# revdotcom/reverb

Hardware: NVIDIA H100
Metric: rtfx_attention_rescoring_30s_chunks (higher is better)
Workload: dtype bf16

## Files before the change

### include/rvb_b200.h

```cpp
#ifndef RVB_B200_H_
#define RVB_B200_H_

#if defined(__GNUC__)
#define RVB_API __attribute__((visibility("default")))
#else
#define RVB_API
#endif

#ifdef __cplusplus
extern "C" {
#endif

typedef struct rvb_model rvb_model;

typedef struct rvb_model_config {
  int input_dim;
  int d_model;
  int heads;
  int ffn_dim;
  int num_blocks;
  int cnn_kernel;
  int causal;
  int cnn_layer_norm;
  int num_langs;
// ... 87 lines not shown
RVB_API int rvb_decoder_step_topk(rvb_model* m, const float* d_enc_out, const int* h_enc_lens, int B, int Tp, int N,
                                  const int* h_hyps, int L, const float* h_cat_embs, int n_cat, int k, float* h_topk_val,
                                  int* h_topk_idx, void* stream);

RVB_API int rvb_decoder_cache_begin(rvb_model* m, const float* d_enc_out, const int* h_enc_lens, int B, int Tp, int N,
                                    int max_steps, const float* h_cat_embs, int n_cat, void* stream);
RVB_API int rvb_decoder_cache_step(rvb_model* m, const int* h_tokens, const int* h_parents, int k, float* h_topk_val,
                                   int* h_topk_idx, void* stream);
RVB_API int rvb_decoder_cache_end(rvb_model* m);

RVB_API int rvb_decoder_step_logp(rvb_model* m, const float* d_enc_out, const int* h_enc_lens, int B, int Tp, int N,
                                  const int* h_hyps, int L, const float* h_cat_embs, int n_cat, float* h_logp,
                                  void* stream);

RVB_API int rvb_ctc_force_align(const float* d_logp, int V, const int* h_enc_lens, int B, int Tp, const int* h_labels,
                                const int* h_label_lens, int max_U, int blank_id, int* h_frames, int* h_first,
                                int* h_last, int* h_peak, float* h_peak_logp, float* h_score, double* h_loglik,
                                void* stream);

typedef struct rvb_aligner rvb_aligner;
RVB_API long long rvb_aligner_workspace_bytes(int U, int total_frames, int want_loglik);
RVB_API rvb_aligner* rvb_aligner_begin(rvb_model* m, const int* h_labels, int U, int total_frames, int V, int blank_id,
                                       int want_loglik, long long budget_bytes, void* stream);
RVB_API int rvb_aligner_push(rvb_aligner* a, const float* d_logp, int n_rows, void* stream);
RVB_API int rvb_aligner_finish(rvb_aligner* a, int* h_frames, int* h_first, int* h_last, int* h_peak, float* h_peak_logp,
                               float* h_score, double* h_loglik, void* stream);
RVB_API void rvb_aligner_abort(rvb_aligner* a);

RVB_API int rvb_gemm_bf16(const void* d_A, const void* d_W, const float* d_bias, int M, int N, int K, int act, int out_mode,
                  float alpha, void* d_out, int ldo, void* stream);
RVB_API int rvb_gemm_bf16_rows(const void* d_A, const void* d_W, const float* d_bias, int M, int N, int K, int act,
                               int out_mode, float alpha, void* d_out, int ldo, const int* d_row_lens, int rows_per_batch,
                               void* stream);
RVB_API int rvb_gemm_bf16x3(const void* d_A, const void* d_W, const float* d_bias, int M, int N, int K, int act, int out_mode,
                            float alpha, void* d_out, int ldo, void* stream);
RVB_API int rvb_gemm_grouped(const void* d_A, const void* d_W, const float* d_bias, int M, int N, int K, int out_mode,
                             void* d_out, int ldo, const int* d_grp, int rows_per_batch, int group_n, int x3,
                             void* stream);
RVB_API int rvb_f32_to_bf16_pair(const float* d_x, void* d_out, long long rows, int width, void* stream);
RVB_API long long rvb_gemm_logsoftmax_gather_ws_bytes(int M, int N);
RVB_API int rvb_gemm_logsoftmax_gather(const void* d_A, const void* d_W, const float* d_bias, int M, int N, int K,
                                       const int* d_gather, void* d_ws, float* d_out, void* stream);
RVB_API int rvb_layernorm(const float* d_x, const float* d_gamma, const float* d_beta, float eps, int M, int d,
                  void* d_out_bf16, float* d_out_f32, void* stream);
RVB_API int rvb_attention(const void* d_q, const void* d_k, const void* d_v, const void* d_p, const float* d_bias_u,
                  const float* d_bias_v, void* d_out, int ldq, int ldk, int ldv, int ldp, int ldo, int Bq, int Tq, int Tk,
                  int H, int dk, int q_per_kv, const int* d_k_lens, const int* d_q_lens, int causal, float scale,
                  void* stream);
RVB_API int rvb_attention_tc(const void* d_q, const void* d_k, const void* d_v, void* d_out, int ldq, int ldk, int ldv,
                             int ldo, int groups, int Tq, int Tk, int H, int dk, const float* d_key_bias,
                             const int* d_k_lens, int causal, float scale, void* stream);
RVB_API int rvb_attention_tc_chunked(const void* d_q, const void* d_k, const void* d_v, void* d_out, int ldq, int ldk,
                                     int ldv, int ldo, int groups, int Tq, int Tk, int H, int dk, const float* d_key_bias,
                                     const int* d_k_lens, int chunk, int left_chunks, float scale, void* stream);
RVB_API int rvb_attention_tc_bits(const void* d_q, const void* d_k, const void* d_v, void* d_out, int ldq, int ldk,
                                  int ldv, int ldo, int groups, int Tq, int Tk, int H, int dk, const float* d_key_bias,
                                  const int* d_k_lens, int causal, const void* d_key_bits, int bits_ld, float scale,
                                  void* stream);
RVB_API int rvb_attention_tc_blocks_per_sm(int Tk, int causal, int chunk, int with_key_bits);
RVB_API int rvb_relpos_prep(const void* d_k, int ldk, const void* d_pos, int ldp, const float* d_bias_u,
                            const float* d_bias_v, void* d_kpp, float* d_cbias, int B, int T, int H, int dk,
                            void* stream);
RVB_API int rvb_f32_to_bf16(const float* d_x, void* d_out, long long n, void* stream);

typedef struct rvb_flac_info {
  int sample_rate;
// ... 30 lines not shown
```

### reverb_b200/_lib.py

```python
from __future__ import annotations

import ctypes as C
import os
from typing import Optional

_HERE = os.path.dirname(os.path.abspath(__file__))
LIB_PATH = os.environ.get("RVB_LIB_PATH") or os.path.join(_HERE, "librvb_b200.so")


class ModelConfig(C.Structure):
    _fields_ = [(n, C.c_int) for n in (
        "input_dim", "d_model", "heads", "ffn_dim", "num_blocks", "cnn_kernel", "causal",
        "cnn_layer_norm", "num_langs", "vocab", "dec_heads", "dec_ffn_dim", "dec_blocks", "r_dec_blocks",
        "sos_id", "eos_id", "precision")]


class SegConfig(C.Structure):
    _fields_ = [(n, C.c_int) for n in (
        "sample_rate", "sinc_filters", "sinc_kernel", "sinc_stride", "conv_channels", "conv_kernel", "lstm_hidden",
        "lstm_layers", "linear_dim", "linear_layers", "num_classes")]


class WavlmSegConfig(C.Structure):
    _fields_ = [(n, C.c_int) for n in (
# ... 40 lines not shown
    "rvb_encoder_forward": (_i, [_vp, _vp, _vp, _i, _i, _vp, _i, _vp, _vp, _vp]),
    "rvb_encoder_forward_chunked": (_i, [_vp, _vp, _vp, _i, _i, _vp, _i, _i, _i, _vp, _vp, _vp]),
    "rvb_encoder_forward_streaming": (_i, [_vp, _vp, _i, _i, _vp, _i, _i, _i, _vp, _vp, _vp]),
    "rvb_ctc_topk": (_i, [_vp, _vp, _i, _i, _i, _f, _i, _vp, _vp, _vp, _vp]),
    "rvb_logp_topk": (_i, [_vp, _i, _i, _i, _vp, _vp, _vp]),
    "rvb_ctc_greedy_search": (_i, [_vp, _i, _vp, _i, _i, _i, _vp, _vp, _vp]),
    "rvb_resample": (_i, [_vp, _i, _ll, _vp, _i, _i, _i, _vp, _ll, _vp]),
    "rvb_ctc_prefix_beam_search": (_i, [_vp, _vp, _i, _vp, _i, _i, _i, _i, _i, _vp, _vp, _vp, _vp, _vp, _vp]),
    "rvb_beam_search_rescoring": (_i, [_vp, _vp, _vp, _i, _vp, _vp, _i, _i, _i, _i, _vp, _i, _f, _i, _vp, _vp, _vp, _vp, _vp,
                                       _vp, _vp, _vp, _vp]),
    "rvb_search_submit": (_i, [_vp, _vp, _vp, _i, _vp, _vp, _i, _i, _i, _i, _vp]),
    "rvb_search_submit_biased": (_i, [_vp, _vp, _vp, _i, _vp, _vp, _i, _i, _i, _i, _vp, _vp]),
    "rvb_context_graph_create": (_vp, [_i, _vp, _vp, _vp, _vp, _vp, _vp, _vp, _i, _i]),
    "rvb_context_graph_destroy": (None, [_vp]),
    "rvb_ctc_prefix_beam_search_biased": (_i, [_vp, _vp, _i, _vp, _i, _i, _i, _i, _i, _vp, _vp, _vp, _vp, _vp, _vp,
                                               _vp]),
    "rvb_rescoring_submit": (_i, [_vp, _i, _vp, _i, _f, _i, _i, _vp, _vp, _vp, _vp, _vp, _vp]),
    "rvb_rescoring_collect": (_i, [_vp, _i, _vp, _vp, _vp]),
    "rvb_ticket_release": (_i, [_vp, _i]),
    "rvb_decoder_step_topk": (_i, [_vp, _vp, _vp, _i, _i, _i, _vp, _i, _vp, _i, _i, _vp, _vp, _vp]),
    "rvb_decoder_cache_begin": (_i, [_vp, _vp, _vp, _i, _i, _i, _i, _vp, _i, _vp]),
    "rvb_decoder_cache_step": (_i, [_vp, _vp, _vp, _i, _vp, _vp, _vp]),
    "rvb_decoder_cache_end": (_i, [_vp]),
    "rvb_decoder_step_logp": (_i, [_vp, _vp, _vp, _i, _i, _i, _vp, _i, _vp, _i, _vp, _vp]),
    "rvb_attention_rescoring": (_i, [_vp, _vp, _vp, _i, _i, _vp, _vp, _i, _i, _vp, _i, _f, _vp, _vp, _vp]),
    "rvb_ctc_force_align": (_i, [_vp, _i, _vp, _i, _i, _vp, _vp, _i, _i, _vp, _vp, _vp, _vp, _vp, _vp, _vp, _vp]),
    "rvb_aligner_workspace_bytes": (_ll, [_i, _i, _i]),
    "rvb_aligner_begin": (_vp, [_vp, _vp, _i, _i, _i, _i, _i, _ll, _vp]),
    "rvb_aligner_push": (_i, [_vp, _vp, _i, _vp]),
    "rvb_aligner_finish": (_i, [_vp, _vp, _vp, _vp, _vp, _vp, _vp, _vp, _vp]),
    "rvb_aligner_abort": (None, [_vp]),
    "rvb_gemm_bf16": (_i, [_vp, _vp, _vp, _i, _i, _i, _i, _i, _f, _vp, _i, _vp]),
    "rvb_gemm_bf16_rows": (_i, [_vp, _vp, _vp, _i, _i, _i, _i, _i, _f, _vp, _i, _vp, _i, _vp]),
    "rvb_gemm_bf16x3": (_i, [_vp, _vp, _vp, _i, _i, _i, _i, _i, _f, _vp, _i, _vp]),
    "rvb_gemm_grouped": (_i, [_vp, _vp, _vp, _i, _i, _i, _i, _vp, _i, _vp, _i, _i, _i, _vp]),
    "rvb_f32_to_bf16_pair": (_i, [_vp, _vp, _ll, _i, _vp]),
    "rvb_gemm_logsoftmax_gather_ws_bytes": (_ll, [_i, _i]),
    "rvb_gemm_logsoftmax_gather": (_i, [_vp, _vp, _vp, _i, _i, _i, _vp, _vp, _vp, _vp]),
    "rvb_layernorm": (_i, [_vp, _vp, _vp, _f, _i, _i, _vp, _vp, _vp]),
    "rvb_attention": (_i, [_vp, _vp, _vp, _vp, _vp, _vp, _vp, _i, _i, _i, _i, _i, _i, _i, _i, _i, _i, _i, _vp, _vp,
                           _i, _f, _vp]),
    "rvb_attention_tc_chunked": (_i, [_vp, _vp, _vp, _vp, _i, _i, _i, _i, _i, _i, _i, _i, _i, _vp, _vp, _i, _i, _f, _vp]),
    "rvb_attention_tc": (_i, [_vp, _vp, _vp, _vp, _i, _i, _i, _i, _i, _i, _i, _i, _i, _vp, _vp, _i, _f, _vp]),
    "rvb_attention_tc_bits": (_i, [_vp, _vp, _vp, _vp, _i, _i, _i, _i, _i, _i, _i, _i, _i, _vp, _vp, _i, _vp, _i, _f,
                                   _vp]),
    "rvb_attention_tc_blocks_per_sm": (_i, [_i, _i, _i, _i]),
    "rvb_relpos_prep": (_i, [_vp, _i, _vp, _i, _vp, _vp, _vp, _vp, _i, _i, _i, _i, _vp]),
    "rvb_f32_to_bf16": (_i, [_vp, _vp, _ll, _vp]),
    "rvb_flac_index_workspace_bytes": (_ll, [_ll]),
    "rvb_flac_index": (_i, [_vp, _ll, _ll, C.POINTER(FlacInfo), _vp, _ll, _vp, _vp, _vp]),
    "rvb_flac_decode_workspace_bytes": (_ll, [_i, _ll, C.POINTER(FlacInfo)]),
    "rvb_flac_decode": (_i, [_vp, _ll, C.POINTER(FlacInfo), _vp, _i, _ll, _vp, _ll, _vp, _vp, _vp, _vp, _vp]),
    "rvb_wav_decode": (_i, [_vp, _ll, C.POINTER(WavCodec), _ll, _vp, _vp, _vp, _vp]),
    "rvb_seg_create": (_vp, [C.POINTER(SegConfig)]),
    "rvb_seg_set_tensor": (_i, [_vp, C.c_char_p, _vp, _ll]),
    "rvb_seg_finalize": (_i, [_vp]),
    "rvb_seg_destroy": (None, [_vp]),
    "rvb_seg_num_frames": (_i, [_vp, _i]),
    "rvb_seg_forward": (_i, [_vp, _vp, _i, _i, _vp, _vp, _vp]),
    "rvb_wavlm_seg_create": (_vp, [C.POINTER(WavlmSegConfig)]),
    "rvb_wavlm_seg_set_tensor": (_i, [_vp, C.c_char_p, _vp, _ll]),
    "rvb_wavlm_seg_finalize": (_i, [_vp]),
    "rvb_wavlm_seg_destroy": (None, [_vp]),
    "rvb_wavlm_seg_num_frames": (_i, [_vp, _i]),
    "rvb_wavlm_seg_forward": (_i, [_vp, _vp, _i, _i, _vp, _vp, _vp, _vp]),
    "rvb_attention_tc_relbias": (_i, [_vp, _vp, _vp, _vp, _i, _i, _i, _i, _i, _i, _i, _vp, _vp, _f, _vp]),
# ... 41 lines not shown
```

### reverb_b200/csrc/engine.cu

```cuda
#include <math.h>
#include <stdarg.h>
#include <stdlib.h>
#include <string.h>

#include <algorithm>
#include <atomic>
#include <memory>
#include <string>
#include <vector>

#include "../../include/rvb_b200.h"
#include "host_mem.h"
#include "kernels.h"

namespace rvb {

static thread_local char g_err[1024] = "";
std::atomic<unsigned long long> g_launch_count{0};
void set_error(const char* fmt, ...) {
  va_list ap;
  va_start(ap, fmt);
  vsnprintf(g_err, sizeof(g_err), fmt, ap);
  va_end(ap);
}
// ... 1881 lines not shown
  g.W = reinterpret_cast<const rvb::bf16*>(d_W);
  g.M = M;
  g.N = N;
  g.K = K;
  g.bias = d_bias;
  g.act = act;
  g.out_mode = out_mode;
  g.alpha = alpha;
  g.out = d_out;
  g.ldo = ldo;
  return rvb::launch_gemm(g, (cudaStream_t)stream);
}

RVB_API int rvb_gemm_bf16_rows(const void* d_A, const void* d_W, const float* d_bias, int M, int N, int K, int act,
                               int out_mode, float alpha, void* d_out, int ldo, const int* d_row_lens, int rows_per_batch,
                               void* stream) {
  rvb::GemmArgs g;
  g.A = reinterpret_cast<const rvb::bf16*>(d_A);
  g.W = reinterpret_cast<const rvb::bf16*>(d_W);
  g.M = M;
  g.N = N;
  g.K = K;
  g.bias = d_bias;
  g.act = act;
  g.out_mode = out_mode;
  g.alpha = alpha;
  g.out = d_out;
  g.ldo = ldo;
  g.row_lens = d_row_lens;
  g.rows_per_batch = rows_per_batch;
  return rvb::launch_gemm(g, (cudaStream_t)stream);
}

RVB_API int rvb_gemm_bf16x3(const void* d_A, const void* d_W, const float* d_bias, int M, int N, int K, int act, int out_mode,
                            float alpha, void* d_out, int ldo, void* stream) {
  rvb::GemmArgs g;
  g.A = reinterpret_cast<const rvb::bf16*>(d_A);
  g.W = reinterpret_cast<const rvb::bf16*>(d_W);
  g.M = M;
  g.N = N;
  g.K = K;
  g.bias = d_bias;
  g.act = act;
  g.out_mode = out_mode;
  g.alpha = alpha;
  g.out = d_out;
  g.ldo = ldo;
  g.x3 = 1;
  if (out_mode == rvb::OUT_BF16) g.out_split = (act == rvb::ACT_GLU) ? N / 2 : N;
  return rvb::launch_gemm(g, (cudaStream_t)stream);
}

RVB_API int rvb_gemm_grouped(const void* d_A, const void* d_W, const float* d_bias, int M, int N, int K, int out_mode,
                             void* d_out, int ldo, const int* d_grp, int rows_per_batch, int group_n, int x3,
                             void* stream) {
  rvb::GemmArgs g;
  g.A = reinterpret_cast<const rvb::bf16*>(d_A);
  g.W = reinterpret_cast<const rvb::bf16*>(d_W);
  g.M = M;
  g.N = N;
  g.K = K;
  g.bias = d_bias;
  g.out_mode = out_mode;
  g.out = d_out;
  g.ldo = ldo;
  g.grp = d_grp;
// ... 138 lines not shown
```

### reverb_b200/csrc/gemm.cu

```cuda
#include <cuda.h>
#include <stdlib.h>
#include <string.h>

#include <algorithm>
#include <mutex>
#include <vector>

#include "kernels.h"

namespace rvb {

static int g_gemm_impl = -1;
void set_gemm_impl(int impl) { g_gemm_impl = impl; }
int get_gemm_impl() {
  if (g_gemm_impl < 0) {
    const char* e = getenv("RVB_GEMM");
    g_gemm_impl = (e && strcmp(e, "simt") == 0) ? 1 : (e && strcmp(e, "narrow") == 0) ? 2 : 0;
  }
  return g_gemm_impl;
}

struct GemmKParams {
  int M, N, K, num_k_blocks;
  int tiles_n, num_tiles;
// ... 232 lines not shown
  }
}

__device__ __forceinline__ long long output_row(const GemmKParams& p, const TileCoord& t, int r) {
  if (p.conv_mode) {
    int tp = t.row0 + r;
    if (tp >= p.conv_T2) return -1;
    return ((long long)t.b * p.conv_T2 + tp) * p.conv_orow_mul + t.f;
  }
  int m = t.row0 + r;
  if (m >= p.M) return -1;
  if (p.row_lens != nullptr) {
    int b = m / p.rows_per_batch;
    int pos = m - b * p.rows_per_batch;
    if (pos >= __ldg(p.row_lens + b)) return -1;
  }
  if (p.grp != nullptr && __ldg(p.grp + m / p.rows_per_batch) != t.g) return -1;
  return m;
}

template <int BN>
__device__ __forceinline__ void acc_ld32(const float* accs, int row, int c, uint32_t* r) {
  const float* rp = accs + row * BN;
#pragma unroll
  for (int k = 0; k < 8; ++k) {
    const float4 v = *reinterpret_cast<const float4*>(rp + ((((c >> 2) + k) ^ (row & 7)) << 2));
    r[4 * k + 0] = __float_as_uint(v.x);
    r[4 * k + 1] = __float_as_uint(v.y);
    r[4 * k + 2] = __float_as_uint(v.z);
    r[4 * k + 3] = __float_as_uint(v.w);
  }
}

template <int BN, int EPI, bool PAIR>
__device__ __forceinline__ void drain_tile(const GemmKParams& p, const TileCoord& t, int q, int lane, const float* accs,
                                           int c0, int c1, float* stage) {
  const int arow = q * 32 + lane;
  const long long orow = output_row(p, t, arow);
  const int n0_tile = t.n0;
  const int oshift = t.g * p.group_n;
  if (p.debug_skip_epi == 1) return;
  if constexpr (EPI == EPI_LSE) {
    const int g = (orow >= 0) ? __ldg(p.lse_gather + orow) : -1;
#pragma unroll 1
    for (int cs = c0; cs < c1; cs += 128) {
      float m = -INFINITY, ssum = 0.f;
#pragma unroll 1
      for (int c = cs; c < cs + 128 && c < c1; c += 32) {
        const int n0 = n0_tile + c;
        if (n0 >= p.N) break;
        uint32_t acc[32];
        acc_ld32<BN>(accs, arow, c, acc);
        float x[32];
        float cm = -INFINITY;
        if (n0 + 32 <= p.N && p.bias != nullptr && (reinterpret_cast<uintptr_t>(p.bias) & 15) == 0) {
          const float2 one2 = make_float2(1.f, 1.f);
          float mx[4] = {-INFINITY, -INFINITY, -INFINITY, -INFINITY};
#pragma unroll
          for (int j = 0; j < 8; ++j) {
            const float4 b4 = __ldg(reinterpret_cast<const float4*>(p.bias + n0) + j);
            const float2 lo = ffma2(make_float2(__uint_as_float(acc[4 * j]), __uint_as_float(acc[4 * j + 1])), one2,
                                    make_float2(b4.x, b4.y));
            const float2 hi = ffma2(make_float2(__uint_as_float(acc[4 * j + 2]), __uint_as_float(acc[4 * j + 3])), one2,
                                    make_float2(b4.z, b4.w));
            x[4 * j] = lo.x;
            x[4 * j + 1] = lo.y;
// ... 159 lines not shown
          float v[8];
          const float2 one2 = make_float2(1.f, 1.f);
#pragma unroll
          for (int h = 0; h < 2; ++h) {
            float4 b4 = make_float4(0.f, 0.f, 0.f, 0.f);
            if (p.bias != nullptr) b4 = __ldg(reinterpret_cast<const float4*>(p.bias + n0) + 2 * j + h);
            float2 lo = ffma2(make_float2(__uint_as_float(acc[8 * j + 4 * h + 0]), __uint_as_float(acc[8 * j + 4 * h + 1])),
                              one2, make_float2(b4.x, b4.y));
            float2 hi = ffma2(make_float2(__uint_as_float(acc[8 * j + 4 * h + 2]), __uint_as_float(acc[8 * j + 4 * h + 3])),
                              one2, make_float2(b4.z, b4.w));
            if (EPI == EPI_BF16_SILU) {
              if constexpr (PAIR) {
                lo = make_float2(lo.x / (1.f + expf(-lo.x)), lo.y / (1.f + expf(-lo.y)));
                hi = make_float2(hi.x / (1.f + expf(-hi.x)), hi.y / (1.f + expf(-hi.y)));
              } else {
                lo = gated2(lo, lo);
                hi = gated2(hi, hi);
              }
            }
            v[4 * h + 0] = lo.x;
            v[4 * h + 1] = lo.y;
            v[4 * h + 2] = hi.x;
            v[4 * h + 3] = hi.y;
          }
          if (EPI == EPI_BF16_RELU) {
#pragma unroll
            for (int e = 0; e < 8; ++e) v[e] = fmaxf(v[e], 0.f);
          }
          if (EPI == EPI_BF16_GELU) {
#pragma unroll
            for (int e = 0; e < 8; ++e) v[e] = gelu_erf(v[e]);
          }
          if constexpr (EPI == EPI_BF16_RELPOS) {
            if (kcols) {
              const uint4 pv = *reinterpret_cast<const uint4*>(p.rp_pos + (long long)rp_t * p.rp_ldp + rp_hc + 8 * j);
              const float4 u0 = __ldg(reinterpret_cast<const float4*>(p.rp_u + rp_hc + 8 * j));
              const float4 u1 = __ldg(reinterpret_cast<const float4*>(p.rp_u + rp_hc + 8 * j) + 1);
              const float uu[8] = {u0.x, u0.y, u0.z, u0.w, u1.x, u1.y, u1.z, u1.w};
              const float4 v0 = __ldg(reinterpret_cast<const float4*>(p.rp_v + rp_hc + 8 * j));
              const float4 v1 = __ldg(reinterpret_cast<const float4*>(p.rp_v + rp_hc + 8 * j) + 1);
              const float2 p0 = unpack_bf16x2(pv.x), p1 = unpack_bf16x2(pv.y), p2 = unpack_bf16x2(pv.z), p3 = unpack_bf16x2(pv.w);
              const float pp[8] = {p0.x, p0.y, p1.x, p1.y, p2.x, p2.y, p3.x, p3.y};
              float kq[8];
#pragma unroll
              for (int e = 0; e < 8; ++e) {
                kq[e] = __bfloat162float(__float2bfloat16(v[e]));
                v[e] = kq[e] + pp[e];
              }
              rp_part[j] = uu[0] * kq[0] + uu[1] * kq[1] + uu[2] * kq[2] + uu[3] * kq[3] + uu[4] * kq[4] + uu[5] * kq[5] +
                           uu[6] * kq[6] + uu[7] * kq[7] + v0.x * pp[0] + v0.y * pp[1] + v0.z * pp[2] + v0.w * pp[3] +
                           v1.x * pp[4] + v1.y * pp[5] + v1.z * pp[6] + v1.w * pp[7];
            }
          }
          if (PAIR && part == 1) {
#pragma unroll
            for (int e = 0; e < 8; ++e) v[e] -= __bfloat162float(__float2bfloat16(v[e]));
          }
          if (p.debug_skip_epi == 3 && v[0] != 123.456f) continue;
          *reinterpret_cast<uint4*>(stage_u + lane * 32 + ((j ^ (lane & 7)) << 2)) =
              make_uint4(pack_bf16x2(v[0], v[1]), pack_bf16x2(v[2], v[3]), pack_bf16x2(v[4], v[5]),
                         pack_bf16x2(v[6], v[7]));
        }
        if (p.debug_skip_epi == 3) continue;
        __syncwarp();
#pragma unroll
        for (int it = 0; it < 8; ++it) {
          const int row = it * 4 + rsub;
          const uint4 u = *reinterpret_cast<const uint4*>(stage_u + row * 32 + ((slot ^ (row & 7)) << 2));
          if (ro[it] >= 0 && p.debug_skip_epi != 2)
            *reinterpret_cast<uint4*>(out + ro[it] + c + (PAIR ? part * p.out_split : 0)) = u;
        }
        __syncwarp();
        }
        if constexpr (EPI == EPI_BF16_RELPOS) {
          if (kcols && orow >= 0) {
            const int hh = rp_hc >> 6;
            p.rp_cb[((orow / p.rp_T) * p.rp_H + hh) * (long long)p.rp_T + rp_t] =
                ((rp_part[0] + rp_part[4]) + (rp_part[2] + rp_part[6])) + ((rp_part[1] + rp_part[5]) + (rp_part[3] + rp_part[7]));
          }
        }
      } else {
        for (int cc = c; cc < c + 64 && cc < c1; cc += 32) {
          if (n0_tile + cc >= p.N) break;
          uint32_t acc[32];
          acc_ld32<BN>(accs, arow, cc, acc);
// ... 208 lines not shown
        if (prev >= 0 && lane == 0) mbar_arrive(&empty[prev]);
        prev = (int)stage;
        if (++stage == STAGES) {
          stage = 0;
          phase ^= 1;
        }
      }
      mbar_arrive(&turn[wg ^ 1]);
      wgmma_wait<0>();
      wgmma_fence_regs<BN>(acc);
      if (prev >= 0 && lane == 0) mbar_arrive(&empty[prev]);
      if (i > 0) mbar_wait(&accfree[wg], hand_parity);
#pragma unroll
      for (int h = 0; h < 2; ++h) {
        const int r0 = h * 64 + wl * 16 + (lane >> 2);
#pragma unroll
        for (int j = 0; j < BN / 8; ++j) {
          const int c = 8 * j + 2 * (lane & 3);
#pragma unroll
          for (int e = 0; e < 2; ++e) {
            const int r = r0 + 8 * e;
            *reinterpret_cast<float2*>(accs + r * BN + ((((c >> 2)) ^ (r & 7)) << 2) + (c & 3)) =
                make_float2(acc[h * (BN / 2) + 4 * j + 2 * e], acc[h * (BN / 2) + 4 * j + 2 * e + 1]);
          }
        }
      }
      asm volatile("bar.sync %0, 128;" ::"r"(1 + wg) : "memory");
      drain_tile<BN, EPI, PAIR>(p, t, wl, lane, accs, 0, BN, stage_w);
      mbar_arrive(&accfree[wg ^ 1]);
    }
  }
}

struct WideCfg {
  static constexpr int BM = 128;
  static constexpr int BN = 256;
  static constexpr int BK = 64;
  static constexpr int STAGES = 3;
  static constexpr uint32_t A_BYTES = BM * BK * 2;
  static constexpr uint32_t B_BYTES = BN * BK * 2;
  static constexpr uint32_t STAGE_BYTES = A_BYTES + B_BYTES;
  static constexpr uint32_t OUT_BYTES = BM * BN * 2;
  static constexpr uint32_t SMEM_BYTES = STAGES * STAGE_BYTES + OUT_BYTES + 256  + 1024 ;
};

template <int EPI>
__global__ void __launch_bounds__(kGemmThreads, 1)
gemm_wide_kernel(const __grid_constant__ CUtensorMap tmA, const __grid_constant__ CUtensorMap tmB, const GemmKParams p) {
  using Cfg = WideCfg;
  constexpr int STAGES = Cfg::STAGES;
  extern __shared__ uint8_t smem_raw[];
  uint8_t* smem = reinterpret_cast<uint8_t*>((reinterpret_cast<uintptr_t>(smem_raw) + 1023) & ~uintptr_t(1023));
  uint8_t* sA = smem;
  uint8_t* sB = smem + STAGES * Cfg::A_BYTES;
  uint8_t* sOut = smem + STAGES * Cfg::STAGE_BYTES;
  uint64_t* bars = reinterpret_cast<uint64_t*>(sOut + Cfg::OUT_BYTES);
  uint64_t* full = bars;
  uint64_t* empty = bars + STAGES;
  uint64_t* ofull = bars + 2 * STAGES;
  uint64_t* ofree = ofull + 1;

  const int warp = threadIdx.x >> 5;
  const int lane = threadIdx.x & 31;

  if (threadIdx.x == 0) {
    for (int i = 0; i < STAGES; ++i) {
      mbar_init(&full[i], 1);
      mbar_init(&empty[i], 8);
    }
    mbar_init(ofull, 256);
    mbar_init(ofree, 96);
    fence_barrier_init();
    tma_prefetch_desc(&tmA);
    tma_prefetch_desc(&tmB);
  }
  __syncthreads();
  const int nkb = p.num_k_blocks;

  if (warp < 4) {
    setmaxnreg_dec<kProducerRegs>();
    if (warp == 0) {
      if (lane == 0) {
        uint32_t stage = 0, phase = 0;
        for (int tile = blockIdx.x; tile < p.num_tiles; tile += gridDim.x) {
          const TileCoord t = decode_tile(p, tile, Cfg::BN);
          for (int kb = 0; kb < nkb; ++kb) {
            mbar_wait(&empty[stage], phase ^ 1);
            mbar_expect_tx(&full[stage], Cfg::STAGE_BYTES);
            if (p.conv_mode) {
              const int tap = kb / p.conv_cblocks;
              const int cb = kb - tap * p.conv_cblocks;
              const int kh = tap / 3, kw = tap - kh * 3;
              tma_load_4d(sA + stage * Cfg::A_BYTES, &tmA, &full[stage], cb * 64, 2 * t.f + kw, t.row0 + (kh >> 1),
                          t.b * 2 + (kh & 1));
            } else {
              tma_load_4d(sA + stage * Cfg::A_BYTES, &tmA, &full[stage], kb * 64, t.row0, 0, 0);
            }
            tma_load_2d(sB + stage * Cfg::B_BYTES, &tmB, &full[stage], kb * 64, t.n0);
            if (++stage == STAGES) {
              stage = 0;
              phase ^= 1;
            }
          }
        }
      }
    } else {
      const int cw = warp - 1;
      const bool store = p.debug_skip_epi == 0;
      bf16* out = reinterpret_cast<bf16*>(p.out);
      int i = 0;
      for (int tile = blockIdx.x; tile < p.num_tiles; tile += gridDim.x, ++i) {
        const TileCoord t = decode_tile(p, tile, Cfg::BN);
        mbar_wait(ofull, i & 1);
        if (store) {
#pragma unroll 4
          for (int r = cw; r < Cfg::BM; r += 3) {
            const long long orow = output_row(p, t, r);
            const uint4 u = *reinterpret_cast<const uint4*>(sOut + r * (Cfg::BN * 2) + ((lane ^ (r & 7)) << 4));
            if (orow >= 0) *reinterpret_cast<uint4*>(out + orow * p.ldo + t.n0 + lane * 8) = u;
          }
        }
        mbar_arrive(ofree);
      }
    }
  } else {
    setmaxnreg_inc<kConsumerRegs>();
    const int wg = (warp >> 2) - 1, wl = warp & 3;
    float acc[Cfg::BN / 2];
    uint32_t stage = 0, phase = 0;
    int i = 0;
    for (int tile = blockIdx.x; tile < p.num_tiles; tile += gridDim.x, ++i) {
      const TileCoord t = decode_tile(p, tile, Cfg::BN);
#pragma unroll
      for (int e = 0; e < Cfg::BN / 2; ++e) acc[e] = 0.f;
      int prev = -1;
      for (int kb = 0; kb < nkb; ++kb) {
        mbar_wait(&full[stage], phase);
        constexpr uint64_t kHalfA = (Cfg::A_BYTES / 2) >> 4;
        const uint64_t adesc = make_sw128_desc(smem_u32(sA + stage * Cfg::A_BYTES)) + wg * kHalfA;
        const uint64_t bdesc = make_sw128_desc(smem_u32(sB + stage * Cfg::B_BYTES));
        wgmma_fence_regs<Cfg::BN / 2>(acc);
        wgmma_fence();
#pragma unroll
        for (int k = 0; k < 4; ++k) wgmma_m64n256k16_ss(acc, adesc + 2 * k, bdesc + 2 * k, 1u);
        wgmma_commit();
        wgmma_wait<1>();
        wgmma_fence_regs<Cfg::BN / 2>(acc);
        if (prev >= 0 && lane == 0) mbar_arrive(&empty[prev]);
        prev = (int)stage;
        if (++stage == STAGES) {
          stage = 0;
          phase ^= 1;
        }
      }
      wgmma_wait<0>();
      wgmma_fence_regs<Cfg::BN / 2>(acc);
      if (lane == 0) mbar_arrive(&empty[prev]);
      if (i > 0) mbar_wait(ofree, (i - 1) & 1);
      if (p.debug_skip_epi != 1) {
        const int r0 = wg * 64 + wl * 16 + (lane >> 2);
        uint32_t* so = reinterpret_cast<uint32_t*>(sOut) + r0 * (Cfg::BN / 2) + (lane & 3);
        const float2 one2 = make_float2(1.f, 1.f);
#pragma unroll
        for (int j = 0; j < Cfg::BN / 8; ++j) {
          float2 b = make_float2(0.f, 0.f);
          if (p.bias != nullptr) b = __ldg(reinterpret_cast<const float2*>(p.bias + t.n0 + 8 * j + 2 * (lane & 3)));
#pragma unroll
          for (int e = 0; e < 2; ++e) {
            float2 v = ffma2(make_float2(acc[4 * j + 2 * e], acc[4 * j + 2 * e + 1]), one2, b);
            if (EPI == EPI_BF16_SILU) v = gated2(v, v);
            if (EPI == EPI_BF16_RELU) v = make_float2(fmaxf(v.x, 0.f), fmaxf(v.y, 0.f));
            so[8 * e * (Cfg::BN / 2) + ((j ^ (lane >> 2)) << 2)] = pack_bf16x2(v.x, v.y);
          }
        }
      }
      mbar_arrive(ofull);
    }
  }
}

__device__ __forceinline__ float load_a_elem(const GemmKParams& p, const TileCoord& t, int r, int k) {
  if (k >= p.K) return 0.0f;
  if (p.conv_mode) {
    int tp = t.row0 + r;
    if (tp >= p.conv_T2) return 0.0f;
    int tap = k / p.conv_C;
    int c = k - tap * p.conv_C;
    int kh = tap / 3, kw = tap - kh * 3;
    long long idx = (((long long)(t.b * 2 + (kh & 1)) * p.conv_T1h + (tp + (kh >> 1))) * p.conv_F1 + (2 * t.f + kw)) *
                        p.conv_C + c;
    return __bfloat162float(p.A[idx]);
  }
  int m = t.row0 + r;
  if (m >= p.M) return 0.0f;
  return __bfloat162float(p.A[(long long)m * p.lda + k]);
}

__global__ void __launch_bounds__(256) gemm_simt_kernel(const GemmKParams p) {
  __shared__ float sA[128][17];
  __shared__ float sW[32][17];
  __shared__ float sG[32][17];
  const bool glu = (p.act == ACT_GLU);
  for (int tile = blockIdx.x; tile < p.num_tiles; tile += gridDim.x) {
    TileCoord t = decode_tile(p, tile, 32);
    const int tx = threadIdx.x & 7, ty = threadIdx.x >> 3;
// ... 115 lines not shown
    cudaEvent_t e;
    RVB_CHECK_CUDA(cudaEventCreate(&e));
    pool.push_back(e);
  }
  *out = pool[g_prof_pool_used[dev]++];
  return 0;
}

void gemm_profile_begin() {
  std::lock_guard<std::mutex> lock(g_prof_mutex);
  g_prof.clear();
  for (int d = 0; d < kProfMaxDev; ++d) g_prof_pool_used[d] = 0;
  g_prof_on = true;
}
int gemm_profile_end(double* total_ms, double* total_flops, long long* launches) {
  g_prof_on = false;
  double ms = 0.0, fl = 0.0;
  for (auto& r : g_prof) {
    float t = 0.f;
    RVB_CHECK_CUDA(cudaEventSynchronize(r.b));
    RVB_CHECK_CUDA(cudaEventElapsedTime(&t, r.a, r.b));
    ms += t;
    fl += r.flops;
  }
  if (total_ms) *total_ms = ms;
  if (total_flops) *total_flops = fl;
  if (launches) *launches = (long long)g_prof.size();
  g_prof.clear();
  return 0;
}

template <int BN>
static int launch_wg(const GemmArgs& a, GemmKParams& p, cudaStream_t stream) {
  constexpr uint32_t SMEM_BYTES = BN == 256 ? WideCfg::SMEM_BYTES : GemmCfg<BN>::SMEM_BYTES;
  CUtensorMap tmA, tmB;
  const int kmul = a.x3 ? 2 : 1;
  const long long lda = a.lda ? a.lda : (long long)a.K * kmul, ldw = a.ldw ? a.ldw : (long long)a.K * kmul;
  if (a.conv_mode) {
    const cuuint64_t Cp = (cuuint64_t)a.conv_C * (a.x3 ? 2 : 1);
    cuuint64_t dims[4] = {Cp, (cuuint64_t)a.conv_F1, (cuuint64_t)a.conv_T1h, (cuuint64_t)(2 * a.conv_B)};
    cuuint64_t str[3] = {Cp * 2, (cuuint64_t)a.conv_F1 * Cp * 2, (cuuint64_t)a.conv_T1h * a.conv_F1 * Cp * 2};
    cuuint32_t box[4] = {64, 1, 128, 1};
    if (make_tmap(&tmA, a.A, 4, dims, str, box)) return -1;
  } else {
    cuuint64_t dims[4] = {(cuuint64_t)a.K * (a.x3 ? 2 : 1), (cuuint64_t)a.M, 1, 1};
    cuuint64_t str[3] = {(cuuint64_t)lda * 2, (cuuint64_t)lda * 2 * a.M, (cuuint64_t)lda * 2 * a.M};
    cuuint32_t box[4] = {64, 128, 1, 1};
    if (make_tmap(&tmA, a.A, 4, dims, str, box)) return -1;
  }
  {
    cuuint64_t dims[2] = {(cuuint64_t)a.K * (a.x3 ? 2 : 1), (cuuint64_t)a.N};
    cuuint64_t str[1] = {(cuuint64_t)ldw * 2};
    cuuint32_t box[2] = {64, (cuuint32_t)BN};
    if (make_tmap(&tmB, a.W, 2, dims, str, box)) return -1;
  }
  void (*kern)(const CUtensorMap, const CUtensorMap, const GemmKParams) = nullptr;
  if constexpr (BN == 256) {
    switch (select_epi(a.act, a.out_mode)) {
      case EPI_BF16: kern = gemm_wide_kernel<EPI_BF16>; break;
      case EPI_BF16_RELU: kern = gemm_wide_kernel<EPI_BF16_RELU>; break;
      default: kern = gemm_wide_kernel<EPI_BF16_SILU>; break;
    }
  } else {
    const bool pair = a.out_split > 0;
    switch (a.rp_pos ? (int)EPI_BF16_RELPOS : select_epi(a.act, a.out_mode)) {
      case EPI_BF16: kern = pair ? gemm_wg_kernel<BN, EPI_BF16, true> : gemm_wg_kernel<BN, EPI_BF16, false>; break;
      case EPI_BF16_RELU: kern = pair ? gemm_wg_kernel<BN, EPI_BF16_RELU, true> : gemm_wg_kernel<BN, EPI_BF16_RELU, false>; break;
      case EPI_BF16_SILU: kern = pair ? gemm_wg_kernel<BN, EPI_BF16_SILU, true> : gemm_wg_kernel<BN, EPI_BF16_SILU, false>; break;
      case EPI_F32: kern = gemm_wg_kernel<BN, EPI_F32, false>; break;
      case EPI_RESID: kern = gemm_wg_kernel<BN, EPI_RESID, false>; break;
      case EPI_GLU: kern = pair ? gemm_wg_kernel<BN, EPI_GLU, true> : gemm_wg_kernel<BN, EPI_GLU, false>; break;
      case EPI_LSE: kern = gemm_wg_kernel<BN, EPI_LSE, false>; break;
      case EPI_BF16_RELPOS: kern = gemm_wg_kernel<BN, EPI_BF16_RELPOS, false>; break;
      case EPI_BF16_GELU: kern = gemm_wg_kernel<BN, EPI_BF16_GELU, false>; break;
      default: kern = gemm_wg_kernel<BN, EPI_GENERIC, false>; break;
    }
  }
  RVB_CHECK_CUDA(cudaFuncSetAttribute(kern, cudaFuncAttributeMaxDynamicSharedMemorySize, (int)SMEM_BYTES));
  p.tiles_n = a.grp ? p.grp_slots * (p.group_n / BN) : (a.N + BN - 1) / BN;
  int tiles_m = a.conv_mode ? a.conv_B * a.conv_F2 * p.conv_tt : (a.M + 127) / 128;
  p.num_tiles = tiles_m * p.tiles_n;
  int grid = p.num_tiles < g_num_sms ? p.num_tiles : g_num_sms;
  GemmProfRec rec;
  if (g_prof_on) {
    if (prof_event(&rec.a) || prof_event(&rec.b)) return -1;
    rec.flops = 2.0 * (double)a.M * (double)(a.grp ? a.group_n : a.N) * (double)a.K * (a.x3 ? 3.0 : 1.0);
    RVB_CHECK_CUDA(cudaEventRecord(rec.a, stream));
  }
  kern<<<grid, kGemmThreads, SMEM_BYTES, stream>>>(tmA, tmB, p);
  RVB_COUNT_LAUNCH();
  RVB_CHECK_LAUNCH();
  if (g_prof_on) {
    RVB_CHECK_CUDA(cudaEventRecord(rec.b, stream));
    {
// ... 112 lines not shown
    p.conv_F1 = a.conv_F1;
    p.conv_C = a.conv_C;
  }
  if (a.out_split > 0)
    RVB_REQUIRE(a.N % 128 == 0 && (a.act == ACT_GLU ? p.glu_coalesced : p.bf16_coalesced),
                "gemm: a hi/lo output pair needs N %% 128 == 0 and 16-byte aligned rows (N=%d)", a.N);
  if (a.act == ACT_GLU) {
    RVB_REQUIRE(a.out_mode == OUT_BF16 && a.N % 64 == 0 && !a.conv_mode, "gemm: ACT_GLU needs bf16 output and N %% 64 == 0");
    RVB_REQUIRE((reinterpret_cast<uintptr_t>(a.out) & 15) == 0 && p.ldo % 8 == 0 &&
                    (a.bias == nullptr || (reinterpret_cast<uintptr_t>(a.bias) & 15) == 0),
                "gemm: ACT_GLU needs 16-byte aligned output rows and bias");
  }
  if (get_gemm_impl() == 1) {
    p.tiles_n = ((a.act == ACT_GLU ? a.N / 2 : a.N) + 31) / 32;
    int tiles_m = a.conv_mode ? a.conv_B * a.conv_F2 * p.conv_tt : (a.M + 127) / 128;
    p.num_tiles = tiles_m * p.tiles_n;
    int grid = p.num_tiles < g_num_sms * 8 ? p.num_tiles : g_num_sms * 8;
    gemm_simt_kernel<<<grid, 256, 0, stream>>>(p);
    RVB_COUNT_LAUNCH();
    RVB_CHECK_LAUNCH();
    return 0;
  }
  RVB_REQUIRE((reinterpret_cast<uintptr_t>(a.A) & 15) == 0 && (reinterpret_cast<uintptr_t>(a.W) & 15) == 0,
              "gemm: operands must be 16-byte aligned");
  RVB_REQUIRE((p.lda * 2) % 16 == 0 && (p.ldw * 2) % 16 == 0, "gemm: leading dimensions must be multiples of 8");
  if (get_encode_fn()) return -1;
  const bool narrow = p.group_n <= 64 || (get_gemm_impl() == 2 && a.out_mode != OUT_LSE && !(a.act == ACT_GLU && a.out_split > 0));
  RVB_REQUIRE(!a.grp || p.group_n % (narrow ? 64 : 128) == 0, "gemm: grouped output needs group_n %% %d == 0 (group_n=%d)",
              narrow ? 64 : 128, p.group_n);
  if (narrow) return launch_wg<64>(a, p, stream);
  const int epi = select_epi(a.act, a.out_mode);
  const long long wide_tiles = (long long)(a.conv_mode ? a.conv_B * a.conv_F2 * p.conv_tt : (a.M + 127) / 128) * (a.N / 256);
  const char* wide_env = getenv("RVB_GEMM_WIDE");
  if ((epi == EPI_BF16 || epi == EPI_BF16_RELU || epi == EPI_BF16_SILU) && !a.rp_pos && !a.grp && !a.x3 &&
      a.out_split == 0 && p.bf16_coalesced && a.N % 256 == 0 && wide_tiles >= g_num_sms &&
      !(wide_env && strcmp(wide_env, "0") == 0))
    return launch_wg<256>(a, p, stream);
  return launch_wg<128>(a, p, stream);
}

}
```

Before: 12910.

## Route relpos and GLU epilogues through the wide 256-column GEMM kernel

Extends the 128x256 wide warp-specialized GEMM kernel to support the relative-position key epilogue and the GLU epilogue. The copy-out warps now apply the positional add and key-bias reduction. GLU halves the output tile in shared memory. Register splits between producer and consumer warps are retuned for these variants. This lets more encoder GEMMs use the larger tile to cut B-operand reloads and tile overhead, at the cost of heavier epilogue work in the producer warpgroup and higher register pressure. A new C API entry point for the relpos GEMM is also added.

```diff
diff --git a/include/rvb_b200.h b/include/rvb_b200.h
--- a/include/rvb_b200.h
+++ b/include/rvb_b200.h
@@ -143,6 +143,9 @@
 RVB_API int rvb_gemm_bf16_rows(const void* d_A, const void* d_W, const float* d_bias, int M, int N, int K, int act,
                                int out_mode, float alpha, void* d_out, int ldo, const int* d_row_lens, int rows_per_batch,
                                void* stream);
+RVB_API int rvb_gemm_bf16_relpos(const void* d_A, const void* d_W, const float* d_bias, int M, int N, int K, void* d_out,
+                                 const void* d_pos, int ldp, int T, int H, int key_col0, const float* d_u, const float* d_v,
+                                 float* d_key_bias, void* stream);
 RVB_API int rvb_gemm_bf16x3(const void* d_A, const void* d_W, const float* d_bias, int M, int N, int K, int act, int out_mode,
                             float alpha, void* d_out, int ldo, void* stream);
 RVB_API int rvb_gemm_grouped(const void* d_A, const void* d_W, const float* d_bias, int M, int N, int K, int out_mode,
diff --git a/reverb_b200/_lib.py b/reverb_b200/_lib.py
--- a/reverb_b200/_lib.py
+++ b/reverb_b200/_lib.py
@@ -96,6 +96,7 @@
     "rvb_aligner_abort": (None, [_vp]),
     "rvb_gemm_bf16": (_i, [_vp, _vp, _vp, _i, _i, _i, _i, _i, _f, _vp, _i, _vp]),
     "rvb_gemm_bf16_rows": (_i, [_vp, _vp, _vp, _i, _i, _i, _i, _i, _f, _vp, _i, _vp, _i, _vp]),
+    "rvb_gemm_bf16_relpos": (_i, [_vp, _vp, _vp, _i, _i, _i, _vp, _vp, _i, _i, _i, _i, _vp, _vp, _vp, _vp]),
     "rvb_gemm_bf16x3": (_i, [_vp, _vp, _vp, _i, _i, _i, _i, _i, _f, _vp, _i, _vp]),
     "rvb_gemm_grouped": (_i, [_vp, _vp, _vp, _i, _i, _i, _i, _vp, _i, _vp, _i, _i, _i, _vp]),
     "rvb_f32_to_bf16_pair": (_i, [_vp, _vp, _ll, _i, _vp]),
diff --git a/reverb_b200/csrc/engine.cu b/reverb_b200/csrc/engine.cu
--- a/reverb_b200/csrc/engine.cu
+++ b/reverb_b200/csrc/engine.cu
@@ -1937,6 +1937,28 @@
   return rvb::launch_gemm(g, (cudaStream_t)stream);
 }
 
+RVB_API int rvb_gemm_bf16_relpos(const void* d_A, const void* d_W, const float* d_bias, int M, int N, int K, void* d_out,
+                                 const void* d_pos, int ldp, int T, int H, int key_col0, const float* d_u, const float* d_v,
+                                 float* d_key_bias, void* stream) {
+  rvb::GemmArgs g;
+  g.A = reinterpret_cast<const rvb::bf16*>(d_A);
+  g.W = reinterpret_cast<const rvb::bf16*>(d_W);
+  g.M = M;
+  g.N = N;
+  g.K = K;
+  g.bias = d_bias;
+  g.out = d_out;
+  g.rp_pos = reinterpret_cast<const rvb::bf16*>(d_pos);
+  g.rp_ldp = ldp;
+  g.rp_T = T;
+  g.rp_H = H;
+  g.rp_col0 = key_col0;
+  g.rp_u = d_u;
+  g.rp_v = d_v;
+  g.rp_cb = d_key_bias;
+  return rvb::launch_gemm(g, (cudaStream_t)stream);
+}
+
 RVB_API int rvb_gemm_bf16x3(const void* d_A, const void* d_W, const float* d_bias, int M, int N, int K, int act, int out_mode,
                             float alpha, void* d_out, int ldo, void* stream) {
   rvb::GemmArgs g;
diff --git a/reverb_b200/csrc/gemm.cu b/reverb_b200/csrc/gemm.cu
--- a/reverb_b200/csrc/gemm.cu
+++ b/reverb_b200/csrc/gemm.cu
@@ -288,6 +288,28 @@
   }
 }
 
+__device__ __forceinline__ float relpos_keys8_pos(const GemmKParams& p, const uint4 pv, int hc, int c8, float* v) {
+  const float4 u0 = __ldg(reinterpret_cast<const float4*>(p.rp_u + hc + c8));
+  const float4 u1 = __ldg(reinterpret_cast<const float4*>(p.rp_u + hc + c8) + 1);
+  const float uu[8] = {u0.x, u0.y, u0.z, u0.w, u1.x, u1.y, u1.z, u1.w};
+  const float4 v0 = __ldg(reinterpret_cast<const float4*>(p.rp_v + hc + c8));
+  const float4 v1 = __ldg(reinterpret_cast<const float4*>(p.rp_v + hc + c8) + 1);
+  const float2 p0 = unpack_bf16x2(pv.x), p1 = unpack_bf16x2(pv.y), p2 = unpack_bf16x2(pv.z), p3 = unpack_bf16x2(pv.w);
+  const float pp[8] = {p0.x, p0.y, p1.x, p1.y, p2.x, p2.y, p3.x, p3.y};
+  float kq[8];
+#pragma unroll
+  for (int e = 0; e < 8; ++e) {
+    kq[e] = __bfloat162float(__float2bfloat16(v[e]));
+    v[e] = kq[e] + pp[e];
+  }
+  return uu[0] * kq[0] + uu[1] * kq[1] + uu[2] * kq[2] + uu[3] * kq[3] + uu[4] * kq[4] + uu[5] * kq[5] +
+         uu[6] * kq[6] + uu[7] * kq[7] + v0.x * pp[0] + v0.y * pp[1] + v0.z * pp[2] + v0.w * pp[3] +
+         v1.x * pp[4] + v1.y * pp[5] + v1.z * pp[6] + v1.w * pp[7];
+}
+__device__ __forceinline__ float relpos_keys8(const GemmKParams& p, int t, int hc, int c8, float* v) {
+  return relpos_keys8_pos(p, *reinterpret_cast<const uint4*>(p.rp_pos + (long long)t * p.rp_ldp + hc + c8), hc, c8, v);
+}
+
 template <int BN, int EPI, bool PAIR>
 __device__ __forceinline__ void drain_tile(const GemmKParams& p, const TileCoord& t, int q, int lane, const float* accs,
                                            int c0, int c1, float* stage) {
@@ -513,25 +535,7 @@
             for (int e = 0; e < 8; ++e) v[e] = gelu_erf(v[e]);
           }
           if constexpr (EPI == EPI_BF16_RELPOS) {
-            if (kcols) {
-              const uint4 pv = *reinterpret_cast<const uint4*>(p.rp_pos + (long long)rp_t * p.rp_ldp + rp_hc + 8 * j);
-              const float4 u0 = __ldg(reinterpret_cast<const float4*>(p.rp_u + rp_hc + 8 * j));
-              const float4 u1 = __ldg(reinterpret_cast<const float4*>(p.rp_u + rp_hc + 8 * j) + 1);
-              const float uu[8] = {u0.x, u0.y, u0.z, u0.w, u1.x, u1.y, u1.z, u1.w};
-              const float4 v0 = __ldg(reinterpret_cast<const float4*>(p.rp_v + rp_hc + 8 * j));
-              const float4 v1 = __ldg(reinterpret_cast<const float4*>(p.rp_v + rp_hc + 8 * j) + 1);
-              const float2 p0 = unpack_bf16x2(pv.x), p1 = unpack_bf16x2(pv.y), p2 = unpack_bf16x2(pv.z), p3 = unpack_bf16x2(pv.w);
-              const float pp[8] = {p0.x, p0.y, p1.x, p1.y, p2.x, p2.y, p3.x, p3.y};
-              float kq[8];
-#pragma unroll
-              for (int e = 0; e < 8; ++e) {
-                kq[e] = __bfloat162float(__float2bfloat16(v[e]));
-                v[e] = kq[e] + pp[e];
-              }
-              rp_part[j] = uu[0] * kq[0] + uu[1] * kq[1] + uu[2] * kq[2] + uu[3] * kq[3] + uu[4] * kq[4] + uu[5] * kq[5] +
-                           uu[6] * kq[6] + uu[7] * kq[7] + v0.x * pp[0] + v0.y * pp[1] + v0.z * pp[2] + v0.w * pp[3] +
-                           v1.x * pp[4] + v1.y * pp[5] + v1.z * pp[6] + v1.w * pp[7];
-            }
+            if (kcols) rp_part[j] = relpos_keys8(p, rp_t, rp_hc, 8 * j, v);
           }
           if (PAIR && part == 1) {
 #pragma unroll
@@ -806,22 +810,27 @@
   }
 }
 
+template <int EPI>
 struct WideCfg {
   static constexpr int BM = 128;
   static constexpr int BN = 256;
   static constexpr int BK = 64;
+  static constexpr int OUT_N = EPI == EPI_GLU ? BN / 2 : BN;
   static constexpr int STAGES = 3;
+  static constexpr bool WIDE_COPY = EPI == EPI_BF16_RELPOS || EPI == EPI_GLU;
+  static constexpr int PRODUCER_REGS = WIDE_COPY ? 88 : kProducerRegs;
+  static constexpr int CONSUMER_REGS = WIDE_COPY ? 208 : kConsumerRegs;
   static constexpr uint32_t A_BYTES = BM * BK * 2;
   static constexpr uint32_t B_BYTES = BN * BK * 2;
   static constexpr uint32_t STAGE_BYTES = A_BYTES + B_BYTES;
-  static constexpr uint32_t OUT_BYTES = BM * BN * 2;
+  static constexpr uint32_t OUT_BYTES = BM * OUT_N * 2;
   static constexpr uint32_t SMEM_BYTES = STAGES * STAGE_BYTES + OUT_BYTES + 256  + 1024 ;
 };
 
 template <int EPI>
 __global__ void __launch_bounds__(kGemmThreads, 1)
 gemm_wide_kernel(const __grid_constant__ CUtensorMap tmA, const __grid_constant__ CUtensorMap tmB, const GemmKParams p) {
-  using Cfg = WideCfg;
+  using Cfg = WideCfg<EPI>;
   constexpr int STAGES = Cfg::STAGES;
   extern __shared__ uint8_t smem_raw[];
   uint8_t* smem = reinterpret_cast<uint8_t*>((reinterpret_cast<uintptr_t>(smem_raw) + 1023) & ~uintptr_t(1023));
@@ -852,7 +861,7 @@
   const int nkb = p.num_k_blocks;
 
   if (warp < 4) {
-    setmaxnreg_dec<kProducerRegs>();
+    setmaxnreg_dec<Cfg::PRODUCER_REGS>();
     if (warp == 0) {
       if (lane == 0) {
         uint32_t stage = 0, phase = 0;
@@ -879,7 +888,9 @@
         }
       }
     } else {
-      const int cw = warp - 1;
+      constexpr int CHUNKS = Cfg::OUT_N / 8;
+      constexpr int RPI = 32 / CHUNKS;
+      const int cw = warp - 1, ch = lane % CHUNKS, rsub = lane / CHUNKS;
       const bool store = p.debug_skip_epi == 0;
       bf16* out = reinterpret_cast<bf16*>(p.out);
       int i = 0;
@@ -887,18 +898,62 @@
         const TileCoord t = decode_tile(p, tile, Cfg::BN);
         mbar_wait(ofull, i & 1);
         if (store) {
+          const int hc = t.n0 + ch * 8 - p.rp_col0;
+          const bool kcol = EPI == EPI_BF16_RELPOS && hc >= 0 && hc < p.rp_H * 64;
+          if (EPI == EPI_BF16_RELPOS && __any_sync(0xffffffffu, kcol)) {
+            constexpr int D = 4;
+#pragma unroll 1
+            for (int r0 = cw; r0 < Cfg::BM; r0 += 3 * D) {
+              int m[D];
+              uint4 pv[D];
+#pragma unroll
+              for (int q = 0; q < D; ++q) {
+                const int r = r0 + 3 * q;
+                m[q] = r < Cfg::BM ? (int)output_row(p, t, r) : -1;
+                pv[q] = make_uint4(0u, 0u, 0u, 0u);
+                if (kcol && m[q] >= 0)
+                  pv[q] = __ldg(reinterpret_cast<const uint4*>(p.rp_pos + (long long)(m[q] % p.rp_T) * p.rp_ldp + hc));
+              }
+#pragma unroll
+              for (int q = 0; q < D; ++q) {
+                const int r = r0 + 3 * q;
+                if (r >= Cfg::BM) break;
+                uint4 u = *reinterpret_cast<const uint4*>(sOut + r * (Cfg::OUT_N * 2) + ((ch ^ (r & 7)) << 4));
+                float part = 0.f;
+                if (kcol && m[q] >= 0) {
+                  const float2 k0 = unpack_bf16x2(u.x), k1 = unpack_bf16x2(u.y), k2 = unpack_bf16x2(u.z),
+                               k3 = unpack_bf16x2(u.w);
+                  float v[8] = {k0.x, k0.y, k1.x, k1.y, k2.x, k2.y, k3.x, k3.y};
+                  part = relpos_keys8_pos(p, pv[q], hc & ~63, hc & 63, v);
+                  u = make_uint4(pack_bf16x2(v[0], v[1]), pack_bf16x2(v[2], v[3]), pack_bf16x2(v[4], v[5]),
+                                 pack_bf16x2(v[6], v[7]));
+                }
+                part += __shfl_xor_sync(0xffffffffu, part, 4);
+                part += __shfl_xor_sync(0xffffffffu, part, 2);
+                part += __shfl_xor_sync(0xffffffffu, part, 1);
+                if (m[q] >= 0) {
+                  if (kcol && (lane & 7) == 0) {
+                    const int rb = m[q] / p.rp_T, rt = m[q] - rb * p.rp_T;
+                    p.rp_cb[((long long)rb * p.rp_H + (hc >> 6)) * p.rp_T + rt] = part;
+                  }
+                  *reinterpret_cast<uint4*>(out + (long long)m[q] * p.ldo + t.n0 + ch * 8) = u;
+                }
+              }
+            }
+          } else {
 #pragma unroll 4
-          for (int r = cw; r < Cfg::BM; r += 3) {
-            const long long orow = output_row(p, t, r);
-            const uint4 u = *reinterpret_cast<const uint4*>(sOut + r * (Cfg::BN * 2) + ((lane ^ (r & 7)) << 4));
-            if (orow >= 0) *reinterpret_cast<uint4*>(out + orow * p.ldo + t.n0 + lane * 8) = u;
+            for (int r = cw * RPI + rsub; r < Cfg::BM; r += 3 * RPI) {
+              const long long orow = output_row(p, t, r);
+              const uint4 u = *reinterpret_cast<const uint4*>(sOut + r * (Cfg::OUT_N * 2) + ((ch ^ (r & 7)) << 4));
+              if (orow >= 0) *reinterpret_cast<uint4*>(out + orow * p.ldo + (EPI == EPI_GLU ? t.n0 / 2 : t.n0) + ch * 8) = u;
+            }
           }
         }
         mbar_arrive(ofree);
       }
     }
   } else {
-    setmaxnreg_inc<kConsumerRegs>();
+    setmaxnreg_inc<Cfg::CONSUMER_REGS>();
     const int wg = (warp >> 2) - 1, wl = warp & 3;
     float acc[Cfg::BN / 2];
     uint32_t stage = 0, phase = 0;
@@ -933,18 +988,40 @@
       if (i > 0) mbar_wait(ofree, (i - 1) & 1);
       if (p.debug_skip_epi != 1) {
         const int r0 = wg * 64 + wl * 16 + (lane >> 2);
-        uint32_t* so = reinterpret_cast<uint32_t*>(sOut) + r0 * (Cfg::BN / 2) + (lane & 3);
+        uint32_t* so = reinterpret_cast<uint32_t*>(sOut) + r0 * (Cfg::OUT_N / 2) + (lane & 3);
         const float2 one2 = make_float2(1.f, 1.f);
-#pragma unroll
-        for (int j = 0; j < Cfg::BN / 8; ++j) {
-          float2 b = make_float2(0.f, 0.f);
-          if (p.bias != nullptr) b = __ldg(reinterpret_cast<const float2*>(p.bias + t.n0 + 8 * j + 2 * (lane & 3)));
-#pragma unroll
-          for (int e = 0; e < 2; ++e) {
-            float2 v = ffma2(make_float2(acc[4 * j + 2 * e], acc[4 * j + 2 * e + 1]), one2, b);
-            if (EPI == EPI_BF16_SILU) v = gated2(v, v);
-            if (EPI == EPI_BF16_RELU) v = make_float2(fmaxf(v.x, 0.f), fmaxf(v.y, 0.f));
-            so[8 * e * (Cfg::BN / 2) + ((j ^ (lane >> 2)) << 2)] = pack_bf16x2(v.x, v.y);
+        if constexpr (EPI == EPI_GLU) {
+#pragma unroll
+          for (int g = 0; g < 4; ++g) {
+#pragma unroll
+            for (int jj = 0; jj < 4; ++jj) {
+              const int j = 8 * g + jj;
+              float2 ba = make_float2(0.f, 0.f), bg = ba;
+              if (p.bias != nullptr) {
+                ba = __ldg(reinterpret_cast<const float2*>(p.bias + t.n0 + 8 * j + 2 * (lane & 3)));
+                bg = __ldg(reinterpret_cast<const float2*>(p.bias + t.n0 + 8 * j + 32 + 2 * (lane & 3)));
+              }
+#pragma unroll
+              for (int e = 0; e < 2; ++e) {
+                const float2 a = ffma2(make_float2(acc[4 * j + 2 * e], acc[4 * j + 2 * e + 1]), one2, ba);
+                const float2 gt = ffma2(make_float2(acc[4 * (j + 4) + 2 * e], acc[4 * (j + 4) + 2 * e + 1]), one2, bg);
+                const float2 v = gated2(a, gt);
+                so[8 * e * (Cfg::OUT_N / 2) + (((4 * g + jj) ^ (lane >> 2)) << 2)] = pack_bf16x2(v.x, v.y);
+              }
+            }
+          }
+        } else {
+#pragma unroll
+          for (int j = 0; j < Cfg::BN / 8; ++j) {
+            float2 b = make_float2(0.f, 0.f);
+            if (p.bias != nullptr) b = __ldg(reinterpret_cast<const float2*>(p.bias + t.n0 + 8 * j + 2 * (lane & 3)));
+#pragma unroll
+            for (int e = 0; e < 2; ++e) {
+              float2 v = ffma2(make_float2(acc[4 * j + 2 * e], acc[4 * j + 2 * e + 1]), one2, b);
+              if (EPI == EPI_BF16_SILU) v = gated2(v, v);
+              if (EPI == EPI_BF16_RELU) v = make_float2(fmaxf(v.x, 0.f), fmaxf(v.y, 0.f));
+              so[8 * e * (Cfg::OUT_N / 2) + ((j ^ (lane >> 2)) << 2)] = pack_bf16x2(v.x, v.y);
+            }
           }
         }
       }
@@ -1126,7 +1203,7 @@
 
 template <int BN>
 static int launch_wg(const GemmArgs& a, GemmKParams& p, cudaStream_t stream) {
-  constexpr uint32_t SMEM_BYTES = BN == 256 ? WideCfg::SMEM_BYTES : GemmCfg<BN>::SMEM_BYTES;
+  uint32_t SMEM_BYTES = GemmCfg<BN>::SMEM_BYTES;
   CUtensorMap tmA, tmB;
   const int kmul = a.x3 ? 2 : 1;
   const long long lda = a.lda ? a.lda : (long long)a.K * kmul, ldw = a.ldw ? a.ldw : (long long)a.K * kmul;
@@ -1150,10 +1227,15 @@
   }
   void (*kern)(const CUtensorMap, const CUtensorMap, const GemmKParams) = nullptr;
   if constexpr (BN == 256) {
-    switch (select_epi(a.act, a.out_mode)) {
-      case EPI_BF16: kern = gemm_wide_kernel<EPI_BF16>; break;
-      case EPI_BF16_RELU: kern = gemm_wide_kernel<EPI_BF16_RELU>; break;
-      default: kern = gemm_wide_kernel<EPI_BF16_SILU>; break;
+    switch (a.rp_pos ? (int)EPI_BF16_RELPOS : select_epi(a.act, a.out_mode)) {
+      case EPI_BF16: kern = gemm_wide_kernel<EPI_BF16>; SMEM_BYTES = WideCfg<EPI_BF16>::SMEM_BYTES; break;
+      case EPI_BF16_RELU: kern = gemm_wide_kernel<EPI_BF16_RELU>; SMEM_BYTES = WideCfg<EPI_BF16_RELU>::SMEM_BYTES; break;
+      case EPI_BF16_SILU: kern = gemm_wide_kernel<EPI_BF16_SILU>; SMEM_BYTES = WideCfg<EPI_BF16_SILU>::SMEM_BYTES; break;
+      case EPI_BF16_RELPOS:
+        kern = gemm_wide_kernel<EPI_BF16_RELPOS>;
+        SMEM_BYTES = WideCfg<EPI_BF16_RELPOS>::SMEM_BYTES;
+        break;
+      default: kern = gemm_wide_kernel<EPI_GLU>; SMEM_BYTES = WideCfg<EPI_GLU>::SMEM_BYTES; break;
     }
   } else {
     const bool pair = a.out_split > 0;
@@ -1332,8 +1414,9 @@
   const int epi = select_epi(a.act, a.out_mode);
   const long long wide_tiles = (long long)(a.conv_mode ? a.conv_B * a.conv_F2 * p.conv_tt : (a.M + 127) / 128) * (a.N / 256);
   const char* wide_env = getenv("RVB_GEMM_WIDE");
-  if ((epi == EPI_BF16 || epi == EPI_BF16_RELU || epi == EPI_BF16_SILU) && !a.rp_pos && !a.grp && !a.x3 &&
-      a.out_split == 0 && p.bf16_coalesced && a.N % 256 == 0 && wide_tiles >= g_num_sms &&
+  const bool wide_epi = epi == EPI_GLU ? p.glu_coalesced
+                                       : (epi == EPI_BF16 || epi == EPI_BF16_RELU || epi == EPI_BF16_SILU) && p.bf16_coalesced;
+  if (wide_epi && !a.grp && !a.x3 && a.out_split == 0 && a.N % 256 == 0 && wide_tiles >= g_num_sms &&
       !(wide_env && strcmp(wide_env, "0") == 0))
     return launch_wg<256>(a, p, stream);
   return launch_wg<128>(a, p, stream);
```

Measured after the change: 12370 (median of 6 runs). 0.958x the previous value.
